# dedis/kyber

Measured on AMD Instinct MI355X. Metric: scalar-muls/s + pairings/s per node; MSM sec at 2^20 points, higher is better.
Workload: dtype int32 limbs (radix 2^25.5), int64 accumulate; 1 GPU; Ed25519 batched fixed-base + var-base scalar-mul, 2^20 scalars per GPU (BASELINE.json configs[1]); elements_per_gpu=1048576

## Files before the change

### kyber_amd/csrc/fe25519.cuh

```cuda
#pragma once
#include "hd.h"

namespace kyb {

struct fe {
    static constexpr int N = 10;
    int32_t v[10];
#if defined(KYB_FE_AUDIT)
    double mag = 2.0;
#endif
};

#if defined(KYB_FE_AUDIT)
inline double& fe_audit_max() {
    static double m = 0;
    return m;
}
inline double& fe_audit_max19() {
    static double m = 0;
    return m;
}
inline void fe_audit_note(double pf, double pg, double scale) {
    const double x = pf * pg * scale;
    if (x > fe_audit_max()) fe_audit_max() = x;
    if (pg > fe_audit_max19()) fe_audit_max19() = pg;
}
#define KYB_FE_MAG_SET(h, x) ((h).mag = (x))
#define KYB_FE_MAG(f) ((f).mag)
#define KYB_FE_NOTE(pf, pg, scale) fe_audit_note(pf, pg, scale)
#else
#define KYB_FE_MAG_SET(h, x) ((void)0)
#define KYB_FE_MAG(f) 0.0
#define KYB_FE_NOTE(pf, pg, scale) ((void)0)
#endif

#if defined(__HIPCC__)
#define KYB_DEV __device__ __forceinline__
#else
#define KYB_DEV inline
#endif

KYB_DEV void fe_0(fe& h) {
#pragma unroll
    for (int i = 0; i < 10; i++) h.v[i] = 0;
    KYB_FE_MAG_SET(h, 0.0);
}
KYB_DEV void fe_1(fe& h) {
    fe_0(h);
    h.v[0] = 1;
    KYB_FE_MAG_SET(h, 1.0 / (1 << 25));
}
KYB_DEV void fe_add(fe& h, const fe& f, const fe& g) {
    const double m_ = KYB_FE_MAG(f) + KYB_FE_MAG(g);
#pragma unroll
    for (int i = 0; i < 10; i++) h.v[i] = f.v[i] + g.v[i];
    KYB_FE_MAG_SET(h, m_);
}
KYB_DEV void fe_sub(fe& h, const fe& f, const fe& g) {
    const double m_ = KYB_FE_MAG(f) + KYB_FE_MAG(g);
#pragma unroll
    for (int i = 0; i < 10; i++) h.v[i] = f.v[i] - g.v[i];
    KYB_FE_MAG_SET(h, m_);
}
KYB_DEV void fe_neg(fe& h, const fe& f) {
    const double m_ = KYB_FE_MAG(f);
#pragma unroll
    for (int i = 0; i < 10; i++) h.v[i] = -f.v[i];
    KYB_FE_MAG_SET(h, m_);
}
KYB_DEV void fe_cmov(fe& f, const fe& g, bool b) {
#pragma unroll
    for (int i = 0; i < 10; i++) f.v[i] = b ? g.v[i] : f.v[i];
    KYB_FE_MAG_SET(f, KYB_FE_MAG(f) > KYB_FE_MAG(g) ? KYB_FE_MAG(f) : KYB_FE_MAG(g));
}
KYB_DEV void fe_cswap(fe& f, fe& g, bool b) {
#pragma unroll
    for (int i = 0; i < 10; i++) {
        int32_t x = f.v[i], y = g.v[i];
        f.v[i] = b ? y : x;
        g.v[i] = b ? x : y;
    }
    const double m_ = KYB_FE_MAG(f) > KYB_FE_MAG(g) ? KYB_FE_MAG(f) : KYB_FE_MAG(g);
    KYB_FE_MAG_SET(f, m_);
    KYB_FE_MAG_SET(g, m_);
    (void)m_;
}

KYB_DEV constexpr int64_t fe_bias(int i) { return (i & 1) ? 0 : ((int64_t)1 << 25) + ((int64_t)1 << 50); }

#if defined(__HIP_DEVICE_COMPILE__)
#define KYB_PIN64(x) asm("" : "+v"(x))
#else
#define KYB_PIN64(x) ((void)0)
#endif
#define KYB_LOW(x, w) ((uint32_t)(x) & ((1u << (w)) - 1u))
#define KYB_CARRY(T, r, i, w)                                        \
    {                                                                \
        const int64_t c_ = (T)[i] >> (w);                            \
        (T)[(i) + 1] += c_;                                          \
        (r)[i] = (int32_t)KYB_LOW((T)[i], w) - (1 << ((w) - 1));     \
    }

KYB_DEV void fe_carry_store(fe& h, int64_t T[10]) {
    int32_t r[10];
    int64_t c = T[0] >> 26;
    T[1] += c;
    const uint32_t b0 = KYB_LOW(T[0], 26);
    KYB_CARRY(T, r, 1, 25);
    KYB_CARRY(T, r, 2, 26);
    KYB_CARRY(T, r, 3, 25);
    KYB_CARRY(T, r, 4, 26);
    KYB_CARRY(T, r, 5, 25);
    KYB_CARRY(T, r, 6, 26);
    KYB_CARRY(T, r, 7, 25);
    KYB_CARRY(T, r, 8, 26);
    c = T[9] >> 25;
    r[9] = (int32_t)KYB_LOW(T[9], 25) - (1 << 24);
    const int64_t t0 = (int64_t)b0 + c * 19;
    c = t0 >> 26;
    r[0] = (int32_t)KYB_LOW(t0, 26) - (1 << 25);
    r[1] += (int32_t)c;
#pragma unroll
    for (int i = 0; i < 10; i++) h.v[i] = r[i];
}

template <class ColF>
KYB_DEV void fe_chain_store(fe& h, ColF col) {
    int32_t r[10];
    const int64_t T0 = col(0, fe_bias(0));
    int64_t c = T0 >> 26;
    const uint32_t b0 = KYB_LOW(T0, 26);
#pragma unroll
    for (int k = 1; k < 10; k++) {
        const int w = (k & 1) ? 25 : 26;
        const int64_t T = (k & 1) ? col(k, c) : col(k, fe_bias(k)) + c;
        c = T >> w;
        r[k] = (int32_t)KYB_LOW(T, w) - (1 << (w - 1));
    }
    const int64_t t0 = (int64_t)b0 + c * 19;
    c = t0 >> 26;
    r[0] = (int32_t)KYB_LOW(t0, 26) - (1 << 25);
    r[1] += (int32_t)c;
#pragma unroll
    for (int i = 0; i < 10; i++) h.v[i] = r[i];
}

KYB_DEV void fe_mul(fe& h, const fe& f, const fe& g) {
    KYB_FE_NOTE(KYB_FE_MAG(f), KYB_FE_MAG(g), 1.0);
    int32_t g19[10], f2[10];
#pragma unroll
    for (int i = 0; i < 10; i++) {
        g19[i] = 19 * g.v[i];
        f2[i] = 2 * f.v[i];
    }
    fe_chain_store(h, [&](int k, int64_t acc) {
#pragma unroll
        for (int i = 0; i < 10; i++) {
            const int j = (k - i + 10) % 10;
            const bool wrap = i > k;
            const bool both_odd = (i & 1) && (j & 1);
            const int32_t a = both_odd ? f2[i] : f.v[i];
            const int32_t b = wrap ? g19[j] : g.v[j];
            acc += (int64_t)a * (int64_t)b;
            KYB_PIN64(acc);
        }
        return acc;
    });
    KYB_FE_MAG_SET(h, 1.01);
}

template <bool DBL>
KYB_DEV void fe_sq_t(fe& h, const fe& f) {
    KYB_FE_NOTE(KYB_FE_MAG(f), KYB_FE_MAG(f), DBL ? 2.0 : 1.0);
    int32_t f2[10], f19[10], f38[10];
#pragma unroll
    for (int i = 0; i < 10; i++) {
        f2[i] = 2 * f.v[i];
        f19[i] = 19 * f.v[i];
        f38[i] = (int32_t)(2u * (uint32_t)f19[i]);
    }
    fe_chain_store(h, [&](int k, int64_t addend) {
        int64_t acc = DBL ? 0 : addend;
#pragma unroll
        for (int i = 0; i < 10; i++) {
            const int j = (k - i + 10) % 10;
            if (i > j) continue;
            const bool wrap = (i + j) >= 10;
            const bool both_odd = (i & 1) && (j & 1);
            const int32_t a = i == j ? f.v[i] : f2[i];
            const int32_t b = wrap ? (both_odd ? f38[j] : f19[j]) : (both_odd ? f2[j] : f.v[j]);
            acc += (int64_t)a * (int64_t)b;
            KYB_PIN64(acc);
        }
        return DBL ? (acc + acc) + addend : acc;
    });
    KYB_FE_MAG_SET(h, 1.01);
}
KYB_DEV void fe_sq_sel(fe& h, const fe& f, bool dbl) {
    KYB_FE_NOTE(KYB_FE_MAG(f), KYB_FE_MAG(f), 2.0);
    fe g = f;
    int32_t f2[10], f19[10], f38[10];
#pragma unroll
    for (int i = 0; i < 10; i++) {
        f2[i] = 2 * g.v[i];
        f19[i] = 19 * g.v[i];
        f38[i] = (int32_t)(2u * (uint32_t)f19[i]);
    }
    int64_t t[10];
#pragma unroll
    for (int k = 0; k < 10; k++) {
        int64_t acc = 0;
#pragma unroll
        for (int i = 0; i < 10; i++) {
            const int j = (k - i + 10) % 10;
            if (i > j) continue;
            const bool wrap = (i + j) >= 10;
            const bool both_odd = (i & 1) && (j & 1);
            const int32_t a = i == j ? g.v[i] : f2[i];
            const int32_t b = wrap ? (both_odd ? f38[j] : f19[j]) : (both_odd ? f2[j] : g.v[j]);
            acc += (int64_t)a * (int64_t)b;
        }
        t[k] = (dbl ? (acc + acc) : acc) + fe_bias(k);
    }
    fe_carry_store(h, t);
    KYB_FE_MAG_SET(h, 1.01);
}
KYB_DEV void fe_sq(fe& h, const fe& f) { fe_sq_t<false>(h, f); }
KYB_DEV void fe_sq2(fe& h, const fe& f) { fe_sq_t<true>(h, f); }

template <class F>
KYB_DEV void fe_sqn(F& h, const F& f, int n) {
    fe_sq(h, f);
#pragma unroll 1
    for (int i = 1; i < n; i++) fe_sq(h, h);
}

template <class F>
KYB_DEV void fe_pow_2_250_1(F& out, F& z11, const F& z) {
    F z2, z9, t, a5, a10, a20, a50, a100;
    fe_sq(z2, z);
    fe_sqn(t, z2, 2);
    fe_mul(z9, t, z);
    fe_mul(z11, z9, z2);
    fe_sq(t, z11);
    fe_mul(a5, t, z9);
    fe_sqn(t, a5, 5);
    fe_mul(a10, t, a5);
    fe_sqn(t, a10, 10);
    fe_mul(a20, t, a10);
    fe_sqn(t, a20, 20);
    fe_mul(t, t, a20);
    fe_sqn(t, t, 10);
    fe_mul(a50, t, a10);
    fe_sqn(t, a50, 50);
    fe_mul(a100, t, a50);
    fe_sqn(t, a100, 100);
    fe_mul(t, t, a100);
    fe_sqn(t, t, 50);
    fe_mul(out, t, a50);
}
template <class F>
KYB_DEV void fe_invert(F& out, const F& z) {
    F t, z11;
    fe_pow_2_250_1(t, z11, z);
    fe_sqn(t, t, 5);
    fe_mul(out, t, z11);
}
template <class F>
KYB_DEV void fe_pow22523(F& out, const F& z) {
    F t, z11;
    fe_pow_2_250_1(t, z11, z);
    fe_sqn(t, t, 2);
    fe_mul(out, t, z);
}

KYB_DEV void fe_towords(uint32_t w[8], const fe& f) {
    int32_t h[10];
#pragma unroll
    for (int i = 0; i < 10; i++) h[i] = f.v[i];
    int32_t q = (19 * h[9] + (1 << 24)) >> 25;
#pragma unroll
    for (int i = 0; i < 10; i++) q = (h[i] + q) >> ((i & 1) ? 25 : 26);
    h[0] += 19 * q;
#pragma unroll
    for (int i = 0; i < 9; i++) {
        const int w_ = (i & 1) ? 25 : 26;
        int32_t c = h[i] >> w_;
        h[i + 1] += c;
        h[i] -= c * (1 << w_);
    }
    h[9] &= (1 << 25) - 1;
    uint32_t u[10];
#pragma unroll
    for (int i = 0; i < 10; i++) u[i] = (uint32_t)h[i];
    w[0] = u[0] | (u[1] << 26);
    w[1] = (u[1] >> 6) | (u[2] << 19);
    w[2] = (u[2] >> 13) | (u[3] << 13);
    w[3] = (u[3] >> 19) | (u[4] << 6);
    w[4] = u[5] | (u[6] << 25);
    w[5] = (u[6] >> 7) | (u[7] << 19);
    w[6] = (u[7] >> 13) | (u[8] << 12);
    w[7] = (u[8] >> 20) | (u[9] << 6);
}
KYB_DEV void fe_fromwords(fe& h, const uint32_t w[8]) {
    h.v[0] = (int32_t)(w[0] & 0x3ffffff);
    h.v[1] = (int32_t)(((w[0] >> 26) | (w[1] << 6)) & 0x1ffffff);
    h.v[2] = (int32_t)(((w[1] >> 19) | (w[2] << 13)) & 0x3ffffff);
    h.v[3] = (int32_t)(((w[2] >> 13) | (w[3] << 19)) & 0x1ffffff);
    h.v[4] = (int32_t)((w[3] >> 6) & 0x3ffffff);
    h.v[5] = (int32_t)(w[4] & 0x1ffffff);
    h.v[6] = (int32_t)(((w[4] >> 25) | (w[5] << 7)) & 0x3ffffff);
    h.v[7] = (int32_t)(((w[5] >> 19) | (w[6] << 13)) & 0x1ffffff);
    h.v[8] = (int32_t)(((w[6] >> 12) | (w[7] << 20)) & 0x3ffffff);
    h.v[9] = (int32_t)((w[7] >> 6) & 0x1ffffff);
    KYB_FE_MAG_SET(h, 2.0);
}
KYB_DEV bool fe_isnegative(const fe& f) {
    uint32_t w[8];
    fe_towords(w, f);
    return w[0] & 1;
}
KYB_DEV bool fe_isnonzero(const fe& f) {
    uint32_t w[8];
    fe_towords(w, f);
    uint32_t r = 0;
#pragma unroll
    for (int i = 0; i < 8; i++) r |= w[i];
    return r != 0;
}

}
```

### kyber_amd/csrc/fe29.cuh

```cuda
#pragma once
#include "fe25519.cuh"

namespace kyb {

struct fe29 {
    static constexpr int N = 9;
    int32_t v[9];
#if defined(KYB_FE_AUDIT)
    double mag = 2.0;
#endif
};

constexpr double FE29_MUL_LIMIT = 14.0;
constexpr double FE29_SQ_LIMIT = 3.99;
constexpr int32_t FE29_MASK = (1 << 29) - 1;
constexpr int32_t FE29_FOLD = 1216;
constexpr int32_t FE29_FOLD_HI = 8 * FE29_FOLD;

#if defined(KYB_FE_AUDIT)
inline double& fe29_audit_max() {
    static double m = 0;
    return m;
}
inline double& fe29_audit_max_sq() {
    static double m = 0;
    return m;
}
inline void fe29_audit_note(double pf, double pg, double scale, bool sq) {
    const double x = pf * pg * scale;
    if (x > fe29_audit_max()) fe29_audit_max() = x;
    if (sq && pf > fe29_audit_max_sq()) fe29_audit_max_sq() = pf;
}
#define KYB_FE29_NOTE(pf, pg, scale, sq) fe29_audit_note(pf, pg, scale, sq)
#else
#define KYB_FE29_NOTE(pf, pg, scale, sq) ((void)0)
#endif

KYB_DEV void fe_0(fe29& h) {
#pragma unroll
    for (int i = 0; i < 9; i++) h.v[i] = 0;
    KYB_FE_MAG_SET(h, 0.0);
}
KYB_DEV void fe_1(fe29& h) {
    fe_0(h);
    h.v[0] = 1;
    KYB_FE_MAG_SET(h, 1.0 / (1 << 28));
}
KYB_DEV void fe_add(fe29& h, const fe29& f, const fe29& g) {
    const double m_ = KYB_FE_MAG(f) + KYB_FE_MAG(g);
#pragma unroll
    for (int i = 0; i < 9; i++) h.v[i] = f.v[i] + g.v[i];
    KYB_FE_MAG_SET(h, m_);
    (void)m_;
}
KYB_DEV void fe_sub(fe29& h, const fe29& f, const fe29& g) {
    const double m_ = KYB_FE_MAG(f) + KYB_FE_MAG(g);
#pragma unroll
    for (int i = 0; i < 9; i++) h.v[i] = f.v[i] - g.v[i];
    KYB_FE_MAG_SET(h, m_);
    (void)m_;
}
KYB_DEV void fe_neg(fe29& h, const fe29& f) {
    const double m_ = KYB_FE_MAG(f);
#pragma unroll
    for (int i = 0; i < 9; i++) h.v[i] = -f.v[i];
    KYB_FE_MAG_SET(h, m_);
    (void)m_;
}
KYB_DEV void fe_cmov(fe29& f, const fe29& g, bool b) {
#pragma unroll
    for (int i = 0; i < 9; i++) f.v[i] = b ? g.v[i] : f.v[i];
    KYB_FE_MAG_SET(f, KYB_FE_MAG(f) > KYB_FE_MAG(g) ? KYB_FE_MAG(f) : KYB_FE_MAG(g));
}
KYB_DEV void fe_cswap(fe29& f, fe29& g, bool b) {
#pragma unroll
    for (int i = 0; i < 9; i++) {
        int32_t x = f.v[i], y = g.v[i];
        f.v[i] = b ? y : x;
        g.v[i] = b ? x : y;
    }
    const double m_ = KYB_FE_MAG(f) > KYB_FE_MAG(g) ? KYB_FE_MAG(f) : KYB_FE_MAG(g);
    KYB_FE_MAG_SET(f, m_);
    KYB_FE_MAG_SET(g, m_);
    (void)m_;
}

KYB_DEV int32_t fe29_fold(int32_t k) {
#if defined(__HIP_DEVICE_COMPILE__)
    asm("" : "+s"(k));
#endif
    return k;
}

KYB_DEV constexpr int64_t fe29_bias(int k) {
    return (k & 1) ? 0 : ((int64_t)1 << 28) + (k < 8 ? ((int64_t)1 << 57) : 0);
}

template <class ProdF>
KYB_DEV void fe29_fold_store(fe29& h, ProdF prod) {
    const int32_t fold = fe29_fold(FE29_FOLD), fold_hi = fe29_fold(FE29_FOLD_HI);
    int32_t r[9];
    int32_t hi = 0;
    int64_t c = 0;
    uint32_t b0 = 0;
#pragma unroll
    for (int k = 0; k < 9; k++) {
        const int64_t H = k < 8 ? prod(k + 9, (int64_t)0) : 0;
        int64_t T = prod(k, (k & 1) ? c : fe29_bias(k));
        if (k < 8) {
            T += (int64_t)((uint64_t)(uint32_t)H * (uint64_t)(uint32_t)fold);
            KYB_PIN64(T);
        }
        if (k > 0) {
            T += (int64_t)hi * (int64_t)fold_hi;
            KYB_PIN64(T);
        }
        if (k > 0 && !(k & 1)) T += c;
        hi = (int32_t)(H >> 32);
        c = T >> 29;
        if (k == 0)
            b0 = (uint32_t)T & (uint32_t)FE29_MASK;
        else
            r[k] = (int32_t)((uint32_t)T & (uint32_t)FE29_MASK) - (1 << 28);
    }
    const int64_t t0 = (int64_t)b0 + c * FE29_FOLD;
    c = t0 >> 29;
    r[0] = (int32_t)((uint32_t)t0 & (uint32_t)FE29_MASK) - (1 << 28);
    r[1] += (int32_t)c;
#pragma unroll
    for (int i = 0; i < 9; i++) h.v[i] = r[i];
}

KYB_DEV void fe_mul(fe29& h, const fe29& f, const fe29& g) {
    KYB_FE29_NOTE(KYB_FE_MAG(f), KYB_FE_MAG(g), 1.0, false);
    fe29_fold_store(h, [&](int k, int64_t acc) {
#pragma unroll
        for (int i = (k > 8 ? k - 8 : 0); i <= (k < 8 ? k : 8); i++) {
            acc += (int64_t)f.v[i] * (int64_t)g.v[k - i];
            KYB_PIN64(acc);
        }
        return acc;
    });
    KYB_FE_MAG_SET(h, 1.001);
}

template <bool DBL>
KYB_DEV void fe29_sq_t(fe29& h, const fe29& f) {
    KYB_FE29_NOTE(KYB_FE_MAG(f), KYB_FE_MAG(f), DBL ? 2.0 : 1.0, true);
    int32_t f2[9];
#pragma unroll
    for (int i = 0; i < 9; i++) f2[i] = 2 * f.v[i];
    fe29_fold_store(h, [&](int k, int64_t acc) {
#pragma unroll
        for (int i = (k > 8 ? k - 8 : 0); 2 * i <= k; i++) {
            const int j = k - i;
            const int32_t a = (i == j && !DBL) ? f.v[i] : f2[i];
            const int32_t b = (i == j || !DBL) ? f.v[j] : f2[j];
            acc += (int64_t)a * (int64_t)b;
            KYB_PIN64(acc);
        }
        return acc;
    });
    KYB_FE_MAG_SET(h, 1.001);
}
KYB_DEV void fe_sq(fe29& h, const fe29& f) { fe29_sq_t<false>(h, f); }
KYB_DEV void fe_sq2(fe29& h, const fe29& f) { fe29_sq_t<true>(h, f); }

KYB_DEV void fe_fromwords(fe29& h, const uint32_t w[8]) {
#pragma unroll
    for (int i = 0; i < 9; i++) {
        const int o = 29 * i, j = o / 32, s = o % 32;
        uint32_t x = w[j] >> s;
        if (s + 29 > 32 && j + 1 < 8) x |= w[j + 1] << (32 - s);
        h.v[i] = (int32_t)(x & (uint32_t)(i < 8 ? FE29_MASK : (1 << 23) - 1));
    }
    KYB_FE_MAG_SET(h, 2.0);
}
KYB_DEV void fe_towords(uint32_t w[8], const fe29& f) {
    int32_t h[9];
#pragma unroll
    for (int i = 0; i < 9; i++) h[i] = f.v[i];
#pragma unroll
    for (int pass = 0; pass < 2; pass++) {
#pragma unroll
        for (int i = 0; i < 8; i++) {
            h[i + 1] += h[i] >> 29;
            h[i] &= FE29_MASK;
        }
        h[0] += 19 * (h[8] >> 23);
        h[8] &= (1 << 23) - 1;
    }
    int32_t q = (h[0] + 19) >> 29;
#pragma unroll
    for (int i = 1; i < 8; i++) q = (h[i] + q) >> 29;
    q = (h[8] + q) >> 23;
    h[0] += 19 * q;
#pragma unroll
    for (int i = 0; i < 8; i++) {
        h[i + 1] += h[i] >> 29;
        h[i] &= FE29_MASK;
    }
    h[8] &= (1 << 23) - 1;
#pragma unroll
    for (int j = 0; j < 8; j++) w[j] = 0;
#pragma unroll
    for (int i = 0; i < 9; i++) {
        const int o = 29 * i, j = o / 32, s = o % 32;
        w[j] |= (uint32_t)h[i] << s;
        if (s + 29 > 32 && j + 1 < 8) w[j + 1] |= (uint32_t)h[i] >> (32 - s);
    }
}
KYB_DEV bool fe_isnegative(const fe29& f) {
    uint32_t w[8];
    fe_towords(w, f);
    return w[0] & 1;
}
KYB_DEV bool fe_isnonzero(const fe29& f) {
    uint32_t w[8];
    fe_towords(w, f);
    uint32_t r = 0;
#pragma unroll
    for (int i = 0; i < 8; i++) r |= w[i];
    return r != 0;
}

KYB_DEV void fe29_to_fe(fe& h, const fe29& f) {
    uint32_t w[8];
    fe_towords(w, f);
    fe_fromwords(h, w);
}
KYB_DEV void fe29_from_fe(fe29& h, const fe& f) {
    uint32_t w[8];
    fe_towords(w, f);
    fe_fromwords(h, w);
}

}
```

### kyber_amd/csrc/ge25519.cuh

```cuda
#pragma once
#include "fe25519.cuh"
#include "fe29.cuh"

namespace kyb {

struct ge_p2 { fe X, Y, Z; };
struct ge_p3 { fe X, Y, Z, T; };
struct ge_p1p1 { fe X, Y, Z, T; };
struct ge_cached { fe YpX, YmX, Z, T2d; };
struct ge_precomp { fe ypx, ymx, xy2d; };
struct ge29_p2 { fe29 X, Y, Z; };
struct ge29_p3 { fe29 X, Y, Z, T; };
struct ge29_p1p1 { fe29 X, Y, Z, T; };
struct ge29_cached { fe29 YpX, YmX, Z, T2d; };
struct ge29_precomp { fe29 ypx, ymx, xy2d; };
template <class F> struct ge_t;
template <> struct ge_t<fe> {
    typedef ge_p2 p2; typedef ge_p3 p3; typedef ge_p1p1 p1p1; typedef ge_cached cached; typedef ge_precomp precomp;
};
template <> struct ge_t<fe29> {
    typedef ge29_p2 p2; typedef ge29_p3 p3; typedef ge29_p1p1 p1p1; typedef ge29_cached cached; typedef ge29_precomp precomp;
};

#include "ed25519_consts.inc"
#include "ed25519_consts29.inc"
template <class F> struct fe_k;
template <> struct fe_k<fe> {
    static KYB_DEV fe d() { return fe_d(); }
    static KYB_DEV fe d2() { return fe_d2(); }
    static KYB_DEV fe sqrtm1() { return fe_sqrtm1(); }
};
template <> struct fe_k<fe29> {
    static KYB_DEV fe29 d() { return fe29_d(); }
    static KYB_DEV fe29 d2() { return fe29_d2(); }
    static KYB_DEV fe29 sqrtm1() { return fe29_sqrtm1(); }
};

template <class P3>
KYB_DEV void ge_p3_0(P3& h) {
    fe_0(h.X);
    fe_1(h.Y);
    fe_1(h.Z);
    fe_0(h.T);
}
template <class C>
KYB_DEV void ge_cached_0(C& c) {
    fe_1(c.YpX);
    fe_1(c.YmX);
    fe_1(c.Z);
    fe_0(c.T2d);
}
template <class P2, class P1>
KYB_DEV void ge_p1p1_to_p2(P2& r, const P1& p) {
    fe_mul(r.X, p.X, p.T);
    fe_mul(r.Y, p.Y, p.Z);
    fe_mul(r.Z, p.Z, p.T);
}
template <class P3, class P1>
KYB_DEV void ge_p1p1_to_p3(P3& r, const P1& p) {
    fe_mul(r.X, p.X, p.T);
    fe_mul(r.Y, p.Y, p.Z);
    fe_mul(r.Z, p.Z, p.T);
    fe_mul(r.T, p.X, p.Y);
}
template <class C, class P3>
KYB_DEV void ge_p3_to_cached(C& r, const P3& p) {
    fe_add(r.YpX, p.Y, p.X);
    fe_sub(r.YmX, p.Y, p.X);
    r.Z = p.Z;
    fe_mul(r.T2d, p.T, fe_k<decltype(p.T)>::d2());
}
template <class P1, class F>
KYB_DEV void ge_dbl(P1& r, const F& X, const F& Y, const F& Z) {
    F t0;
    fe_sq(r.X, X);
    fe_sq(r.Z, Y);
    fe_sq2(r.T, Z);
    fe_add(r.Y, X, Y);
    fe_sq(t0, r.Y);
    fe_add(r.Y, r.Z, r.X);
    fe_sub(r.Z, r.Z, r.X);
    fe_sub(r.X, t0, r.Y);
    fe_sub(r.T, r.T, r.Z);
}
template <class F>
KYB_DEV void ge_cached_xy(F& X, F& Y, const F& YpX, const F& YmX) {
#pragma unroll
    for (int l = 0; l < F::N; l++) {
        X.v[l] = (YpX.v[l] - YmX.v[l]) >> 1;
        Y.v[l] = (YpX.v[l] + YmX.v[l]) >> 1;
    }
    KYB_FE_MAG_SET(X, KYB_FE_MAG(YpX) > KYB_FE_MAG(YmX) ? KYB_FE_MAG(YpX) : KYB_FE_MAG(YmX));
    KYB_FE_MAG_SET(Y, KYB_FE_MAG(X));
}
template <class P1, class C>
KYB_DEV void ge_dbl_cached(P1& r, const C& q) {
    decltype(q.Z) x, y, t0;
    ge_cached_xy(x, y, q.YpX, q.YmX);
    fe_sq(r.X, x);
    fe_sq(r.Z, y);
    fe_sq2(r.T, q.Z);
    fe_sq(t0, q.YpX);
    fe_add(r.Y, r.Z, r.X);
    fe_sub(r.Z, r.Z, r.X);
    fe_sub(r.X, t0, r.Y);
    fe_sub(r.T, r.T, r.Z);
}
template <class P1, class C>
KYB_DEV void ge_cached_to_p1p1(P1& r, const C& q) {
    ge_cached_xy(r.X, r.Y, q.YpX, q.YmX);
    r.Z = q.Z;
    r.T = q.Z;
}
template <class P3, class C>
KYB_DEV void ge_precomp_to_p3(P3& r, const C& q) {
    fe_sub(r.X, q.ypx, q.ymx);
    fe_add(r.Y, q.ypx, q.ymx);
    fe_0(r.Z);
    r.Z.v[0] = 2;
    KYB_FE_MAG_SET(r.Z, 2.0 / (1 << 25));
    fe_mul(r.T, q.xy2d, fe_dinv());
}
template <class P1, class P3, class C>
KYB_DEV void ge_add(P1& r, const P3& p, const C& q) {
    decltype(p.X) t0;
    fe_add(r.X, p.Y, p.X);
    fe_sub(r.Y, p.Y, p.X);
    fe_mul(r.Z, r.X, q.YpX);
    fe_mul(r.Y, r.Y, q.YmX);
    fe_mul(r.T, q.T2d, p.T);
    fe_mul(r.X, p.Z, q.Z);
    fe_add(t0, r.X, r.X);
    fe_sub(r.X, r.Z, r.Y);
    fe_add(r.Y, r.Z, r.Y);
    fe_add(r.Z, t0, r.T);
    fe_sub(r.T, t0, r.T);
}
template <class P1, class P3, class C>
KYB_DEV void ge_madd(P1& r, const P3& p, const C& q) {
    decltype(p.X) t0;
    fe_add(r.X, p.Y, p.X);
    fe_sub(r.Y, p.Y, p.X);
    fe_mul(r.Z, r.X, q.ypx);
    fe_mul(r.Y, r.Y, q.ymx);
    fe_mul(r.T, q.xy2d, p.T);
    fe_add(t0, p.Z, p.Z);
    fe_sub(r.X, r.Z, r.Y);
    fe_add(r.Y, r.Z, r.Y);
    fe_add(r.Z, t0, r.T);
    fe_sub(r.T, t0, r.T);
}
template <class C>
KYB_DEV void ge_cached_cneg(C& c, bool neg) {
    fe_cswap(c.YpX, c.YmX, neg);
    decltype(c.T2d) nt;
    fe_neg(nt, c.T2d);
    fe_cmov(c.T2d, nt, neg);
}
KYB_DEV void ge_precomp_cneg(ge_precomp& c, bool neg) {
    fe_cswap(c.ypx, c.ymx, neg);
    fe nt;
    fe_neg(nt, c.xy2d);
    fe_cmov(c.xy2d, nt, neg);
}

template <class F>
KYB_DEV void ge_encode_with_zinv(uint32_t w[8], const F& X, const F& Y, const F& zinv) {
    F x, y;
    fe_mul(x, X, zinv);
    fe_mul(y, Y, zinv);
    fe_towords(w, y);
    w[7] ^= (uint32_t)fe_isnegative(x) << 31;
}
template <class P3>
KYB_DEV void ge_p3_towords(uint32_t w[8], const P3& p) {
    decltype(p.Z) zi;
    fe_invert(zi, p.Z);
    ge_encode_with_zinv(w, p.X, p.Y, zi);
}
template <class P3>
KYB_DEV bool ge_p3_fromwords(P3& p, const uint32_t w[8]) {
    typedef decltype(p.X) F;
    F u, v, v3, vxx, check;
    fe_fromwords(p.Y, w);
    fe_1(p.Z);
    fe_sq(u, p.Y);
    fe_mul(v, u, fe_k<F>::d());
    fe_sub(u, u, p.Z);
    fe_add(v, v, p.Z);
    fe_sq(v3, v);
    fe_mul(v3, v3, v);
    fe_sq(p.X, v3);
    fe_mul(p.X, p.X, v);
    fe_mul(p.X, p.X, u);
    fe_pow22523(p.X, p.X);
    fe_mul(p.X, p.X, v3);
    fe_mul(p.X, p.X, u);
    fe_sq(vxx, p.X);
    fe_mul(vxx, vxx, v);
    fe_sub(check, vxx, u);
    bool ok = true;
    if (fe_isnonzero(check)) {
        fe_add(check, vxx, u);
        ok = !fe_isnonzero(check);
        F xs;
        fe_mul(xs, p.X, fe_k<F>::sqrtm1());
        p.X = xs;
    }
    const bool sign = (w[7] >> 31) != 0;
    F nx;
    fe_neg(nx, p.X);
    fe_cmov(p.X, nx, fe_isnegative(p.X) != sign);
    fe_mul(p.T, p.X, p.Y);
    return ok;
}

KYB_DEV void recode16(int8_t e[65], const uint32_t a[8], bool full256) {
    int carry = 0;
#pragma unroll
    for (int i = 0; i < 64; i++) {
        int d = (int)((a[i >> 3] >> ((i & 7) * 4)) & 15) + carry;
        if (i < 63) {
            carry = (d + 8) >> 4;
            d -= carry << 4;
        }
        e[i] = (int8_t)d;
    }
    int top = e[63];
    int c2 = 0;
    if (full256) {
        c2 = (top + 8) >> 4;
        top -= c2 << 4;
    } else if (top > 8) {
        top = 0;
    }
    e[63] = (int8_t)top;
    e[64] = (int8_t)c2;
}

KYB_DEV bool ed_effective_scalar(uint32_t (&k)[8]) {
    uint32_t c = 0, t7 = 0;
#pragma unroll
    for (int j = 0; j < 8; j++) {
        const uint64_t s = (uint64_t)k[j] + (j < 7 ? 0x88888888u : 0x08888888u) + c;
        t7 = (uint32_t)s;
        c = (uint32_t)(s >> 32);
    }
    const uint32_t e63 = (c << 4) | (t7 >> 28);
    if (e63 <= 8) return false;
    const uint32_t carried = e63 - (k[7] >> 28);
    k[7] &= 0x0fffffffu;
    if (!carried) return false;
    uint32_t b = 0;
#pragma unroll
    for (int j = 0; j < 8; j++) {
        const uint64_t d = (uint64_t)(j == 7 ? 0x10000000u : 0u) - k[j] - b;
        k[j] = (uint32_t)d;
        b = (uint32_t)(d >> 63);
    }
    return true;
}

}
```

Before: 200.6 million scalar-muls/s.

## Interleave independent fe29 multiplications and fold bias constants into precomputed offsets

Adds paired field-multiply/square routines that run two independent 9-limb product and carry chains step by step together, exposing instruction-level parallelism. The group add, double and conversion formulas now call these pairs. The per-column bias is also recomputed into a constexpr scheme, with an a0 offset plus beta terms folded through the high columns, checked by static_assert. This removes the per-column bias constants. Pinning now uses an SGPR token instead of pinning each 64-bit accumulator. The risks are higher register pressure and lower occupancy from the doubled live state. There is a potential aliasing hazard in ge_add, where r.Y is both an input and an output of the pair, though the chain reads inputs before the final store.

After: 200.3 million scalar-muls/s (median of 2 runs). About the same (-0.1%).

```diff
diff --git a/kyber_amd/csrc/fe25519.cuh b/kyber_amd/csrc/fe25519.cuh
--- a/kyber_amd/csrc/fe25519.cuh
+++ b/kyber_amd/csrc/fe25519.cuh
@@ -227,6 +227,23 @@
 }
 KYB_DEV void fe_sq(fe& h, const fe& f) { fe_sq_t<false>(h, f); }
 KYB_DEV void fe_sq2(fe& h, const fe& f) { fe_sq_t<true>(h, f); }
+KYB_DEV void fe_mul_pair(fe& h1, const fe& f1, const fe& g1, fe& h2, const fe& f2, const fe& g2) {
+    fe_mul(h1, f1, g1);
+    fe_mul(h2, f2, g2);
+}
+KYB_DEV void fe_sq_pair(fe& h1, const fe& f1, fe& h2, const fe& f2) {
+    fe_sq(h1, f1);
+    fe_sq(h2, f2);
+}
+KYB_DEV void fe_sq2_sq_pair(fe& h1, const fe& f1, fe& h2, const fe& f2) {
+    fe_sq2(h1, f1);
+    fe_sq(h2, f2);
+}
+KYB_DEV void fe_sq2_sqsum_pair(fe& h1, const fe& f1, fe& h2, fe& s, const fe& f, const fe& g) {
+    fe_sq2(h1, f1);
+    fe_add(s, f, g);
+    fe_sq(h2, s);
+}
 
 template <class F>
 KYB_DEV void fe_sqn(F& h, const F& f, int n) {
diff --git a/kyber_amd/csrc/fe29.cuh b/kyber_amd/csrc/fe29.cuh
--- a/kyber_amd/csrc/fe29.cuh
+++ b/kyber_amd/csrc/fe29.cuh
@@ -85,86 +85,159 @@
     (void)m_;
 }
 
-KYB_DEV int32_t fe29_fold(int32_t k) {
+#ifndef KYB_FE29_FAULT
+#define KYB_FE29_FAULT 0
+#endif
+
+struct fe29_bias_t {
+    int64_t a0;
+    int64_t beta[8];
+};
+constexpr fe29_bias_t fe29_bias_make() {
+    const int64_t U = (int64_t)1 << 28;
+    int64_t d[9] = {0, 0, U, U, U, U, U, U, U};
+    int64_t r = 0;
+    for (int k = 8; k >= 0; k--) r = ((r << 29) + d[k]) % FE29_FOLD;
+    d[0] -= r;
+    int64_t q[9] = {}, rem = 0;
+    for (int k = 8; k >= 0; k--) {
+        const int64_t cur = (rem << 29) + d[k];
+        q[k] = cur / FE29_FOLD;
+        rem = cur % FE29_FOLD;
+    }
+    fe29_bias_t b = {U + (U << 29) + r, {q[0], q[1], q[2], q[3], q[4], q[5], q[6], q[7] + (q[8] << 29)}};
+#if KYB_FE29_FAULT == 1
+    b.beta[7] = 0;
+#elif KYB_FE29_FAULT == 2
+    b.a0 -= r;
+#endif
+    return b;
+}
+constexpr bool fe29_bias_holds(const fe29_bias_t& b) {
+    int64_t c = 0;
+    for (int k = 0; k < 9; k++) {
+        const int64_t v = c + (k == 0 ? b.a0 : 0) + (k < 8 ? FE29_FOLD * b.beta[k] : 0);
+        if ((v & FE29_MASK) != ((int64_t)1 << 28)) return false;
+        c = v >> 29;
+    }
+    return c == 0;
+}
+constexpr fe29_bias_t FE29_BIAS = fe29_bias_make();
+#if !KYB_FE29_FAULT
+static_assert(fe29_bias_holds(FE29_BIAS), "a0 + 1216 * sum beta_j 2^(29 (j - 9)) = 2^28 * sum 2^(29 k)");
+static_assert(FE29_BIAS.a0 > 0 && FE29_BIAS.beta[7] < ((int64_t)1 << 47), "the bound of a high column counts on it");
+#else
+static_assert(!fe29_bias_holds(FE29_BIAS) || KYB_FE29_FAULT == 3, "a faulted build has to break the identity");
+#endif
+
 #if defined(__HIP_DEVICE_COMPILE__)
-    asm("" : "+s"(k));
-#endif
-    return k;
-}
-
-KYB_DEV constexpr int64_t fe29_bias(int k) {
-    return (k & 1) ? 0 : ((int64_t)1 << 28) + (k < 8 ? ((int64_t)1 << 57) : 0);
-}
-
-template <class ProdF>
-KYB_DEV void fe29_fold_store(fe29& h, ProdF prod) {
-    const int32_t fold = fe29_fold(FE29_FOLD), fold_hi = fe29_fold(FE29_FOLD_HI);
+#define KYB_FE29_PIN(x, tok) asm("" : "+s"(tok) : "v"(x))
+#else
+#define KYB_FE29_PIN(x, tok) ((void)(tok))
+#endif
+struct fe29_chain {
     int32_t r[9];
     int32_t hi = 0;
     int64_t c = 0;
     uint32_t b0 = 0;
-#pragma unroll
-    for (int k = 0; k < 9; k++) {
-        const int64_t H = k < 8 ? prod(k + 9, (int64_t)0) : 0;
-        int64_t T = prod(k, (k & 1) ? c : fe29_bias(k));
-        if (k < 8) {
-            T += (int64_t)((uint64_t)(uint32_t)H * (uint64_t)(uint32_t)fold);
-            KYB_PIN64(T);
-        }
-        if (k > 0) {
-            T += (int64_t)hi * (int64_t)fold_hi;
-            KYB_PIN64(T);
-        }
-        if (k > 0 && !(k & 1)) T += c;
+    int32_t fold = FE29_FOLD, fold_hi = FE29_FOLD_HI, shift = 29;
+    template <class ProdF>
+    KYB_DEV void step(int k, const ProdF& prod) {
+        const int64_t H = k < 8 ? prod(k + 9, FE29_BIAS.beta[k < 8 ? k : 0], fold) : 0;
+#if KYB_FE29_FAULT == 3
+        int64_t T = prod(k, k == 0 ? FE29_BIAS.a0 : k == 4 ? ((int64_t)1 << 28) + ((int64_t)1 << 57) : c, k == 0 ? fold : fold_hi);
+#else
+        int64_t T = prod(k, k == 0 ? FE29_BIAS.a0 : c, k == 0 ? fold : fold_hi);
+#endif
+        if (k < 8) T += (int64_t)((uint64_t)(uint32_t)H * (uint64_t)(uint32_t)fold);
+        if (k > 0 && k < 8) KYB_FE29_PIN(T, shift);
+        if (k > 0) T += (int64_t)hi * (int64_t)fold_hi;
         hi = (int32_t)(H >> 32);
-        c = T >> 29;
+        c = T >> shift;
         if (k == 0)
             b0 = (uint32_t)T & (uint32_t)FE29_MASK;
         else
             r[k] = (int32_t)((uint32_t)T & (uint32_t)FE29_MASK) - (1 << 28);
     }
-    const int64_t t0 = (int64_t)b0 + c * FE29_FOLD;
-    c = t0 >> 29;
-    r[0] = (int32_t)((uint32_t)t0 & (uint32_t)FE29_MASK) - (1 << 28);
-    r[1] += (int32_t)c;
-#pragma unroll
-    for (int i = 0; i < 9; i++) h.v[i] = r[i];
-}
-
-KYB_DEV void fe_mul(fe29& h, const fe29& f, const fe29& g) {
-    KYB_FE29_NOTE(KYB_FE_MAG(f), KYB_FE_MAG(g), 1.0, false);
-    fe29_fold_store(h, [&](int k, int64_t acc) {
+    KYB_DEV void store(fe29& h) {
+        const int64_t t0 = (int64_t)b0 + c * FE29_FOLD;
+        c = t0 >> 29;
+        r[0] = (int32_t)((uint32_t)t0 & (uint32_t)FE29_MASK) - (1 << 28);
+        r[1] += (int32_t)c;
+#pragma unroll
+        for (int i = 0; i < 9; i++) h.v[i] = r[i];
+        KYB_FE_MAG_SET(h, 1.001);
+    }
+};
+template <class ProdF>
+KYB_DEV void fe29_fold_store(fe29& h, const ProdF& prod) {
+    fe29_chain A;
+#pragma unroll
+    for (int k = 0; k < 9; k++) A.step(k, prod);
+    A.store(h);
+}
+template <class Prod1, class Prod2>
+KYB_DEV void fe29_fold_store_pair(fe29& h1, const Prod1& prod1, fe29& h2, const Prod2& prod2) {
+    fe29_chain A, B;
+#pragma unroll
+    for (int k = 0; k < 9; k++) {
+        A.step(k, prod1);
+        B.step(k, prod2);
+    }
+    A.store(h1);
+    B.store(h2);
+}
+
+struct fe29_mul_cols {
+    const fe29 &f, &g;
+    KYB_DEV fe29_mul_cols(const fe29& f_, const fe29& g_) : f(f_), g(g_) { KYB_FE29_NOTE(KYB_FE_MAG(f), KYB_FE_MAG(g), 1.0, false); }
+    KYB_DEV int64_t operator()(int k, int64_t acc, int32_t& tok) const {
 #pragma unroll
         for (int i = (k > 8 ? k - 8 : 0); i <= (k < 8 ? k : 8); i++) {
             acc += (int64_t)f.v[i] * (int64_t)g.v[k - i];
-            KYB_PIN64(acc);
+            KYB_FE29_PIN(acc, tok);
         }
         return acc;
-    });
-    KYB_FE_MAG_SET(h, 1.001);
-}
-
+    }
+};
 template <bool DBL>
-KYB_DEV void fe29_sq_t(fe29& h, const fe29& f) {
-    KYB_FE29_NOTE(KYB_FE_MAG(f), KYB_FE_MAG(f), DBL ? 2.0 : 1.0, true);
+struct fe29_sq_cols {
+    const fe29& f;
     int32_t f2[9];
-#pragma unroll
-    for (int i = 0; i < 9; i++) f2[i] = 2 * f.v[i];
-    fe29_fold_store(h, [&](int k, int64_t acc) {
+    KYB_DEV explicit fe29_sq_cols(const fe29& f_) : f(f_) {
+        KYB_FE29_NOTE(KYB_FE_MAG(f), KYB_FE_MAG(f), DBL ? 2.0 : 1.0, true);
+#pragma unroll
+        for (int i = 0; i < 9; i++) f2[i] = 2 * f.v[i];
+    }
+    KYB_DEV int64_t operator()(int k, int64_t acc, int32_t& tok) const {
 #pragma unroll
         for (int i = (k > 8 ? k - 8 : 0); 2 * i <= k; i++) {
             const int j = k - i;
             const int32_t a = (i == j && !DBL) ? f.v[i] : f2[i];
             const int32_t b = (i == j || !DBL) ? f.v[j] : f2[j];
             acc += (int64_t)a * (int64_t)b;
-            KYB_PIN64(acc);
+            KYB_FE29_PIN(acc, tok);
         }
         return acc;
-    });
-    KYB_FE_MAG_SET(h, 1.001);
-}
-KYB_DEV void fe_sq(fe29& h, const fe29& f) { fe29_sq_t<false>(h, f); }
-KYB_DEV void fe_sq2(fe29& h, const fe29& f) { fe29_sq_t<true>(h, f); }
+    }
+};
+
+KYB_DEV void fe_mul(fe29& h, const fe29& f, const fe29& g) { fe29_fold_store(h, fe29_mul_cols(f, g)); }
+KYB_DEV void fe_sq(fe29& h, const fe29& f) { fe29_fold_store(h, fe29_sq_cols<false>(f)); }
+KYB_DEV void fe_sq2(fe29& h, const fe29& f) { fe29_fold_store(h, fe29_sq_cols<true>(f)); }
+KYB_DEV void fe_mul_pair(fe29& h1, const fe29& f1, const fe29& g1, fe29& h2, const fe29& f2, const fe29& g2) {
+    fe29_fold_store_pair(h1, fe29_mul_cols(f1, g1), h2, fe29_mul_cols(f2, g2));
+}
+KYB_DEV void fe_sq_pair(fe29& h1, const fe29& f1, fe29& h2, const fe29& f2) {
+    fe29_fold_store_pair(h1, fe29_sq_cols<false>(f1), h2, fe29_sq_cols<false>(f2));
+}
+KYB_DEV void fe_sq2_sq_pair(fe29& h1, const fe29& f1, fe29& h2, const fe29& f2) {
+    fe29_fold_store_pair(h1, fe29_sq_cols<true>(f1), h2, fe29_sq_cols<false>(f2));
+}
+KYB_DEV void fe_sq2_sqsum_pair(fe29& h1, const fe29& f1, fe29& h2, fe29& s, const fe29& f, const fe29& g) {
+    fe_add(s, f, g);
+    fe_sq2_sq_pair(h1, f1, h2, s);
+}
 
 KYB_DEV void fe_fromwords(fe29& h, const uint32_t w[8]) {
 #pragma unroll
diff --git a/kyber_amd/csrc/ge25519.cuh b/kyber_amd/csrc/ge25519.cuh
--- a/kyber_amd/csrc/ge25519.cuh
+++ b/kyber_amd/csrc/ge25519.cuh
@@ -52,16 +52,13 @@
 }
 template <class P2, class P1>
 KYB_DEV void ge_p1p1_to_p2(P2& r, const P1& p) {
-    fe_mul(r.X, p.X, p.T);
-    fe_mul(r.Y, p.Y, p.Z);
+    fe_mul_pair(r.X, p.X, p.T, r.Y, p.Y, p.Z);
     fe_mul(r.Z, p.Z, p.T);
 }
 template <class P3, class P1>
 KYB_DEV void ge_p1p1_to_p3(P3& r, const P1& p) {
-    fe_mul(r.X, p.X, p.T);
-    fe_mul(r.Y, p.Y, p.Z);
-    fe_mul(r.Z, p.Z, p.T);
-    fe_mul(r.T, p.X, p.Y);
+    fe_mul_pair(r.X, p.X, p.T, r.Y, p.Y, p.Z);
+    fe_mul_pair(r.Z, p.Z, p.T, r.T, p.X, p.Y);
 }
 template <class C, class P3>
 KYB_DEV void ge_p3_to_cached(C& r, const P3& p) {
@@ -73,11 +70,8 @@
 template <class P1, class F>
 KYB_DEV void ge_dbl(P1& r, const F& X, const F& Y, const F& Z) {
     F t0;
-    fe_sq(r.X, X);
-    fe_sq(r.Z, Y);
-    fe_sq2(r.T, Z);
-    fe_add(r.Y, X, Y);
-    fe_sq(t0, r.Y);
+    fe_sq_pair(r.X, X, r.Z, Y);
+    fe_sq2_sqsum_pair(r.T, Z, t0, r.Y, X, Y);
     fe_add(r.Y, r.Z, r.X);
     fe_sub(r.Z, r.Z, r.X);
     fe_sub(r.X, t0, r.Y);
@@ -97,10 +91,8 @@
 KYB_DEV void ge_dbl_cached(P1& r, const C& q) {
     decltype(q.Z) x, y, t0;
     ge_cached_xy(x, y, q.YpX, q.YmX);
-    fe_sq(r.X, x);
-    fe_sq(r.Z, y);
-    fe_sq2(r.T, q.Z);
-    fe_sq(t0, q.YpX);
+    fe_sq_pair(r.X, x, r.Z, y);
+    fe_sq2_sq_pair(r.T, q.Z, t0, q.YpX);
     fe_add(r.Y, r.Z, r.X);
     fe_sub(r.Z, r.Z, r.X);
     fe_sub(r.X, t0, r.Y);
@@ -126,10 +118,8 @@
     decltype(p.X) t0;
     fe_add(r.X, p.Y, p.X);
     fe_sub(r.Y, p.Y, p.X);
-    fe_mul(r.Z, r.X, q.YpX);
-    fe_mul(r.Y, r.Y, q.YmX);
-    fe_mul(r.T, q.T2d, p.T);
-    fe_mul(r.X, p.Z, q.Z);
+    fe_mul_pair(r.Z, r.X, q.YpX, r.Y, r.Y, q.YmX);
+    fe_mul_pair(r.T, q.T2d, p.T, r.X, p.Z, q.Z);
     fe_add(t0, r.X, r.X);
     fe_sub(r.X, r.Z, r.Y);
     fe_add(r.Y, r.Z, r.Y);
```
